# sjz5202/DisenLink

Measured on AMD Instinct MI355X. Metric: edges/sec (aggregate+score) at K=8 d=64, higher is better.
Workload: dtype f32; 1 GPU; squirrel_real (edge list of the parity fixture)(seed 0): N=5201, edge rows=217073, 85/5/10 split, E_sym=342129, scored train pairs P=1009603 (m=5), K=8, d=64, beta=0.5, t=1.0; forward route+aggregate+score_pairs; K=8, d=64, n_nodes=5201, E_sym=342129, P=1009603

## Files before the change

disenlink_amd/_lib.py:

```python
from __future__ import annotations

import ctypes as C
import os

PKG = os.path.dirname(os.path.abspath(__file__))
LIB_PATH = os.path.join(PKG, "libdisenlink_hip.so")


class DlCsrPlan(C.Structure):
    _fields_ = [
        ("n_rows", C.c_int32), ("row_offset", C.c_int32), ("n_total", C.c_int32), ("n_entries", C.c_int32),
        ("rowptr", C.c_void_p), ("col", C.c_void_p),
        ("seg_len", C.c_int32), ("n_seg", C.c_int32),
        ("seg_row", C.c_void_p), ("seg_beg", C.c_void_p), ("seg_end", C.c_void_p), ("seg_slot", C.c_void_p),
        ("n_slices", C.c_int32), ("slice_max_seg", C.c_int32), ("slice_seg0", C.c_void_p),
        ("n_multi", C.c_int32), ("n_slots", C.c_int32), ("multi_row", C.c_void_p), ("multi_slot0", C.c_void_p),
        ("slot_multi", C.c_void_p), ("unit_count", C.c_void_p),
    ]


class DlPairHub(C.Structure):
    _fields_ = [("n_blocks", C.c_int32), ("block_row", C.c_void_p),
                ("n_items", C.c_int32), ("n_slices", C.c_int32), ("slice_max_item", C.c_int32),
                ("slice_item0", C.c_void_p), ("item_block", C.c_void_p), ("item_step", C.c_void_p),
                ("n_steps", C.c_int32), ("step_v", C.c_void_p), ("step_u", C.c_void_p), ("step_q", C.c_void_p),
                ("step_q2", C.c_void_p), ("n_entries", C.c_int32),
                ("rest", DlCsrPlan), ("rest_pair", C.c_void_p), ("rest_pair2", C.c_void_p)]


class DlGraph(C.Structure):
    _fields_ = [("csr", DlCsrPlan), ("route", DlCsrPlan), ("rev", C.c_void_p), ("route_mirror", C.c_int32),
                ("route_hub", C.POINTER(DlPairHub))]


class DlPairIncidence(C.Structure):
    _fields_ = [("csr", DlCsrPlan), ("inc_pair", C.c_void_p), ("n_pairs", C.c_int32), ("entry_yw", C.c_void_p),
                ("inc_pair2", C.c_void_p), ("n_second", C.c_int32), ("hub", C.POINTER(DlPairHub))]


class DlHostCsr(C.Structure):
    _fields_ = [("n_nodes", C.c_int32), ("n_entries", C.c_int32), ("rowptr", C.POINTER(C.c_int32)),
                ("col", C.POINTER(C.c_int32)), ("rev", C.POINTER(C.c_int32))]


class DlHostPlan(C.Structure):
    _fields_ = [(n, C.c_int32) for n in ("seg_len", "n_seg", "n_slices", "slice_max_seg", "n_multi", "n_slots")] + \
               [(n, C.POINTER(C.c_int32)) for n in ("seg_row", "seg_beg", "seg_end", "seg_slot", "slice_seg0",
                                                    "multi_row", "multi_slot0", "slot_multi")]


class DlSparseFeatures(C.Structure):
    _fields_ = [("N", C.c_int32), ("F", C.c_int32), ("nnz", C.c_int32),
# ... 306 lines not shown
```

disenlink_amd/csrc/dl_api.hip:

```cpp
#include <stdarg.h>
#include <string.h>
#include "dl_common.h"
#include "dl_kernels.h"

namespace dl {

static thread_local char g_err[512] = "";
static int g_force_generic = 0;

void set_error(const char* fmt, ...) {
    va_list ap;
    va_start(ap, fmt);
    vsnprintf(g_err, sizeof(g_err), fmt, ap);
    va_end(ap);
}

int check_launch(const char* what) {
    hipError_t e = hipGetLastError();
    if (e != hipSuccess) {
        set_error("%s: %s", what, hipGetErrorString(e));
        return DL_E_LAUNCH;
    }
    return DL_OK;
}
// ... 258 lines not shown
static int score_pairs_fwd_space(const void* Z, const void* H, int N, int K, int d, dl_dtype dtype, float t,
                                 const int32_t* pu, const int32_t* pv, int n_pairs, const dl_pair_incidence* by_u,
                                 float* prob, float* coef, bool logit, void* stream) {
    if (int rc = check_shape(K, d)) return rc;
    if (int rc = check_dtype(by_u ? &by_u->csr : nullptr, K, d, dtype)) return rc;
    DL_REQUIRE(N >= 0 && n_pairs >= 0, "negative size");
    DL_REQUIRE(t != 0.0f, "temperature is 0");
    if (n_pairs == 0) return DL_OK;
    DL_REQUIRE(Z && H && pu && pv && prob, "NULL argument");
    if (by_u) {
        if (int rc = check_plan(&by_u->csr, "by_u")) return rc;
        const int n_second = by_u->inc_pair2 ? by_u->n_second : 0;
        DL_REQUIRE(n_second >= 0 && by_u->csr.n_entries + n_second == n_pairs && by_u->n_pairs == n_pairs && by_u->inc_pair,
                   "by_u must list each of the %d pairs exactly once", n_pairs);
        DL_REQUIRE(by_u->csr.n_total == N, "by_u.n_total=%d != N=%d", by_u->csr.n_total, N);
        if (const dl_pair_hub* hp = by_u->hub) {
            DL_REQUIRE(hp->n_items >= 0 && hp->n_entries >= 0 && hp->rest.n_entries >= 0 &&
                       hp->n_entries + hp->rest.n_entries == by_u->csr.n_entries,
                       "by_u.hub must hold each of the plan's %d entries exactly once", by_u->csr.n_entries);
            if (int rc = hp->n_items > 0 ? check_hub(hp, "by_u.hub", by_u->inc_pair2 != nullptr) : DL_OK) return rc;
            if (hp->rest.n_entries > 0) {
                if (int rc = check_plan(&hp->rest, "by_u.hub.rest")) return rc;
                DL_REQUIRE(hp->rest.n_total == N && hp->rest.seg_len == by_u->csr.seg_len && hp->rest_pair &&
                           (hp->rest_pair2 || !by_u->inc_pair2), "by_u.hub.rest does not match by_u");
            }
        }
        if (use_fast(&by_u->csr, K, d, dtype))
            return logit ? fast_score_pairs_logits_fwd(by_u, Z, H, K, d, dtype, t, prob, (hipStream_t)stream)
                         : fast_score_pairs_fwd(by_u, Z, H, K, d, dtype, t, prob, coef, (hipStream_t)stream);
    }
    DL_REQUIRE(coef == nullptr, "coef output needs the tuned scorer (a (K,d) with a fast path and a by_u plan)");
    if (logit)
        return generic_score_pairs_logits_fwd((const float*)Z, (const float*)H, K, d, t, pu, pv, n_pairs, prob,
                                              (hipStream_t)stream);
    return generic_score_pairs_fwd((const float*)Z, (const float*)H, K, d, t, pu, pv, n_pairs, prob,
                                   (hipStream_t)stream);
}

int dl_score_pairs_fwd(const void* Z, const void* H, int N, int K, int d, dl_dtype dtype, float t,
// ... 954 lines not shown
```

disenlink_amd/csrc/dl_config.h:

```cpp
#pragma once

namespace dl {

struct Config {
    int stream_rows;
    bool fwd_group_kernel;
    bool fwd_hub;
    bool route_hub;
    int auc_target;
    bool project_fp32_mfma;
    int fwd_groups;
    long long fwd_block_rows;
    long long bwd_block_bytes;
    int bwd_target;
    int inkernel_combine;
    int rank_slices;
    int mine_tiles;
    int sparse_seg;
};

const Config& config();
void config_reload();

}
// ... 1 lines not shown
```

disenlink_amd/csrc/dl_config.hip:

```cpp
#include <stdlib.h>
#include <algorithm>
#include <mutex>
#include "dl_config.h"
#include "disenlink_hip.h"

namespace dl {
namespace {

Config g_config;
std::once_flag g_once;

bool flag(const char* name) {
    const char* e = getenv(name);
    return e != nullptr && e[0] != '\0' && !(e[0] == '0' && e[1] == '\0');
}
long long number(const char* name) {
    const char* e = getenv(name);
    return e != nullptr && e[0] != '\0' ? atoll(e) : 0;
}

void read_environment() {
    Config c;
    const char* sr = getenv("DL_STREAM_ROWS");
    c.stream_rows = (sr == nullptr || sr[0] == '\0') ? -1 : (sr[0] == '1' ? 1 : 0);
    c.fwd_group_kernel = flag("DL_FWD_GROUP_KERNEL");
    const char* fh = getenv("DL_FWD_HUB");
    c.fwd_hub = !(fh != nullptr && fh[0] == '0' && fh[1] == '\0');
    const char* rh = getenv("DL_ROUTE_HUB");
    c.route_hub = !(rh != nullptr && rh[0] == '0' && rh[1] == '\0');
    c.auc_target = (int)std::max(0LL, number("DL_AUC_TARGET"));
    c.project_fp32_mfma = getenv("DL_PROJECT_FP32_MFMA") != nullptr;
    c.fwd_groups = (int)std::max(0LL, number("DL_FWD_GROUPS"));
    c.fwd_block_rows = std::max(0LL, number("DL_FWD_BLOCK_ROWS"));
    c.bwd_block_bytes = std::max(0LL, number("DL_BWD_BLOCK_BYTES"));
    c.bwd_target = (int)std::max(0LL, number("DL_BWD_TARGET"));
    const char* ic = getenv("DL_INKERNEL_COMBINE");
    c.inkernel_combine = (ic == nullptr || ic[0] == '\0') ? 1 : std::max(0, std::min(2, atoi(ic)));
    c.rank_slices = (int)std::max(0LL, number("DL_RANK_SLICES"));
    c.mine_tiles = (int)std::max(0LL, std::min(1LL << 20, number("DL_MINE_TILES")));
    c.sparse_seg = (int)std::max(0LL, std::min(1LL << 20, number("DL_SPARSE_SEG")));
    g_config = c;
}

}
// ... 15 lines not shown
```

disenlink_amd/csrc/dl_hub.h:

```cpp
#pragma once
#include "dl_fast.h"

namespace dl::fast::hub {
constexpr int WAVES = 8, THREADS = WAVES * DL_WAVE;
static_assert(DL_HUB_W == 2 * WAVES, "every wave stages two rows of the block");

typedef int dl_vi4 __attribute__((ext_vector_type(4)));
__device__ __forceinline__ dl_vi4 plan_words(const int32_t* a, int idx) {
    const auto* g = (const __attribute__((address_space(1))) int32_t*)a;
    return reinterpret_cast<const __attribute__((address_space(4))) dl_vi4*>((const __attribute__((address_space(4))) int32_t*)g)[idx];
}

template <bool ONE_STREAM>
__device__ __forceinline__ bool workgroup_item(const dl_pair_hub& h, int& it) {
    it = (int)blockIdx.x;
    if (ONE_STREAM && h.n_slices == 1) return it < h.n_items;
    const int x = blockIdx.x % h.n_slices;
    it = h.slice_item0[x] + (int)(blockIdx.x / h.n_slices);
    return it < h.slice_item0[x + 1];
}

struct ItemSteps { int a, b, c, end; };
__device__ __forceinline__ ItemSteps item_steps(const dl_pair_hub& h, int it) {
    return {h.item_step[4 * it], h.item_step[4 * it + 1], h.item_step[4 * it + 2], h.item_step[4 * it + 3]};
// ... 13 lines not shown
#pragma unroll
            for (int n = 0; n < NTAB; ++n) x[n] = dl_vf4{0.0f, 0.0f, 0.0f, 0.0f};
            if (row >= 0) {
#pragma unroll
                for (int n = 0; n < NTAB; ++n)
                    x[n] = *reinterpret_cast<const dl_vf4*>(tab[n] + (size_t)row * (NJ * 256) + (j * 64 + lane) * 4);
            }
#pragma unroll
            for (int n = 0; n < NTAB; ++n) urow[(ul * NTAB + n) * (NJ * 64) + j * 64 + lane] = x[n];
        }
    }
}

using FULL = std::false_type;
using LAST = std::true_type;
constexpr std::integral_constant<int, 4> SHAPE_A{};
constexpr std::integral_constant<int, 2> SHAPE_B{};
constexpr std::integral_constant<int, 1> SHAPE_C{};
template <typename Words, typename Fetch, typename Step>
__device__ __forceinline__ void walk(int s, const ItemSteps& st, Words nxt, Fetch&& fetch, Step&& step) {
    auto take = [&](const int cur) {
        const Words w = nxt;
        if (cur + WAVES < st.end) nxt = fetch(cur + WAVES);
        return w;
    };
    for (; s < st.b - 1; s += WAVES) step(take(s), s, SHAPE_A, FULL{});
    if (s == st.b - 1) step(take(s), s, SHAPE_A, LAST{}), s += WAVES;
    for (; s < st.c - 1; s += WAVES) step(take(s), s, SHAPE_B, FULL{});
    if (s == st.c - 1) step(take(s), s, SHAPE_B, LAST{}), s += WAVES;
    for (; s < st.end; s += WAVES) step(take(s), s, SHAPE_C, FULL{});
}

template <int NB, bool RARE_FLUSH>
struct Batch {
    int nb = 0;
    template <typename Flush, typename Open>
    __device__ __forceinline__ void tick(int step, Flush&& flush, Open&& open) {
        if (RARE_FLUSH ? __builtin_expect(nb == NB, 0) : nb == NB) {
            flush(), nb = 0, open(step + WAVES);
        }
    }
    template <typename Flush>
    __device__ __forceinline__ void close(Flush&& flush) { if (nb > 0) flush(); }
};
// ... 2 lines not shown
```

disenlink_amd/csrc/dl_score.h:

```cpp
#pragma once
#include "dl_fast.h"
#include "dl_hub.h"
#include "dl_score_bwd.h"

namespace dl {
namespace fast {

template <int K, int D, typename T, bool COEF, bool LOGIT = false>
__global__ __launch_bounds__(BLOCK, K <= 8 ? 4 : 1) void score_fwd_seg_kernel(dl_csr_plan g, const int32_t* __restrict__ pair_id,
                                                              const int32_t* __restrict__ pair_id2,
                                                              const T* __restrict__ Z, const T* __restrict__ H,
                                                              float t, float* __restrict__ prob,
                                                              float* __restrict__ coef_e,
                                                              float* __restrict__ coef_q) {
    using GE = Geo<K, D, T>;
    constexpr int VEC = GE::VEC, G = GE::G, EPW = GE::EPW, ROW = GE::ROW;
    constexpr int KB = K > 8 ? 8 : K;
    using FLB = FactorLanes<G, KB>;
    constexpr int KBP = FLB::KP;
    __shared__ __attribute__((aligned(16))) float urow[WAVES_PER_BLOCK][2 * ROW];
    const WaveSeg ws = load_wave_seg(g);
    const SegInfo si = ws.si;
    const int wave = ws.wave, lane = lane_id();
    const bool active = ws.active;
// ... 188 lines not shown
                 "v_add_f32_dpp %1, %5, %5 row_shl:4 row_mask:0xf bank_mask:0x5\n\t"
                 "v_add_f32_dpp %2, %6, %6 row_shl:4 row_mask:0xf bank_mask:0x5\n\t"
                 "v_add_f32_dpp %3, %7, %7 row_shl:4 row_mask:0xf bank_mask:0x5\n\t"
                 "v_add_f32_dpp %0, %8, %8 row_shr:4 row_mask:0xf bank_mask:0xa\n\t"
                 "v_add_f32_dpp %1, %9, %9 row_shr:4 row_mask:0xf bank_mask:0xa\n\t"
                 "v_add_f32_dpp %2, %10, %10 row_shr:4 row_mask:0xf bank_mask:0xa\n\t"
                 "v_add_f32_dpp %3, %11, %11 row_shr:4 row_mask:0xf bank_mask:0xa\n\t"
                 "s_nop 1"
                 : "=&v"(b[0]), "=&v"(b[1]), "=&v"(b[2]), "=&v"(b[3])
                 : "v"(a[0]), "v"(a[1]), "v"(a[2]), "v"(a[3]), "v"(a[4]), "v"(a[5]), "v"(a[6]), "v"(a[7]));
#pragma unroll
    for (int q = 0; q < 4; ++q) v[q] = b[q];
    TransposedReduce<4, 2>::run(v, c);
}

template <int K, int D, bool T1, bool COEF, bool FOLD, bool LOGIT = false>
__global__ __launch_bounds__(THREADS) __attribute__((amdgpu_waves_per_eu(4, 4))) void score_fwd_wave_kernel(
    dl_pair_hub h, const float* __restrict__ Z, const float* __restrict__ H, float t, float* __restrict__ prob,
    float* __restrict__ coef_e, float* __restrict__ coef_q) {
    using FW = FwdWave<K, D>;
    constexpr int NJ = FW::NJ, U = FW::U, ROW = K * D, R4 = 2 * ROW / 4;
    static_assert(D == 64 && NJ >= 1 && U == 4 && U * NJ <= 8, "the step geometry of score_fwd_wave_kernel");
    static_assert(!(LOGIT && COEF), "the logit form has no stored terms");
    constexpr bool BATCH = !COEF;
    __shared__ __attribute__((aligned(16))) float4 urow[DL_HUB_W * R4];
    int it;
    if (!workgroup_item<false>(h, it)) return;
    const int wave = wave_index(), lane = lane_id();
    const int i = lane & 15, r = lane >> 4;
    const int blk = h.item_block[it];
    const ItemSteps st = item_steps(h, it);
    stage_block<NJ, 2>((lds_vf4*)urow, h, blk, wave, lane, {Z, H});
    __syncthreads();
    auto fetch = [&](const int step) {
        const int s = __builtin_amdgcn_readfirstlane(step);
        StepWords w;
        w.v = plan_words(h.step_v, s), w.u = plan_words(h.step_u, s);
        w.q = w.p = dl_vi4{-1, -1, -1, -1};
        if constexpr (!BATCH) {
            w.q = plan_words(h.step_q, s);
            if constexpr (FOLD) w.p = plan_words(h.step_q2, s);
        }
        return w;
    };
    const int slot_step = lane >> 2;
    float lg = 0.0f;
// ... 1 lines not shown
    Batch<16, true> batch;
    auto open = [&](const int s0) {
        const int sb = s0 + WAVES * slot_step;
        pq = pq2 = -1;
        if (sb < st.end) {
            pq = h.step_q[4 * sb + (lane & 3)];
            if constexpr (FOLD) pq2 = h.step_q2[4 * sb + (lane & 3)];
        }
    };
    auto flush = [&]() {
        const float p = LOGIT ? lg : sigmoid_ref(lg);
        if (pq >= 0) prob[pq] = p;
        if (FOLD && pq2 >= 0) prob[pq2] = p;
    };
    auto do_step = [&](const StepWords& w, auto shape, auto last) {
        constexpr int NV = decltype(shape)::value;
        constexpr bool LAST = decltype(last)::value;
        const int sv[4] = {w.v.x, w.v.y, w.v.z, w.v.w}, su[4] = {w.u.x, w.u.y, w.u.z, w.u.w}, sq[4] = {w.q.x, w.q.y, w.q.z, w.q.w},
                  sq2[4] = {w.p.x, w.p.y, w.p.z, w.p.w};
        float4 zv[NV][NJ], hv[NV][NJ];
#pragma unroll
        for (int n = 0; n < NV; ++n) {
            if (!LAST || sv[n] >= 0) {
                const size_t v = (size_t)(unsigned)sv[n];
                const auto* zr = uniform_row<dl_vf4>(Z, v * ROW * sizeof(float));
                const auto* hr = uniform_row<dl_vf4>(H, v * ROW * sizeof(float));
#pragma unroll
                for (int j = 0; j < NJ; ++j) {
                    zv[n][j] = as_float4(zr[(unsigned)(lane + j * 64)]);
                    hv[n][j] = as_float4(hr[(unsigned)(lane + j * 64)]);
                }
// ... 4 lines not shown
        }
        float val[16];
#pragma unroll
        for (int q = 0; q < 16; ++q) val[q] = 0.0f;
#pragma unroll
        for (int j = 0; j < NJ; ++j) {
            float4 a4[U], b4[U];
#pragma unroll
            for (int e = 0; e < U; ++e) {
                const float4* mine = urow + (su[e] & (DL_HUB_W - 1)) * R4;
                a4[e] = mine[j * 64 + lane], b4[e] = mine[ROW / 4 + j * 64 + lane];
            }
            __builtin_amdgcn_sched_barrier(0);
#pragma unroll
            for (int e = 0; e < U; ++e) {
                val[j * 4 + e] = dot4_packed(a4[e], zv[e * NV / 4][j]);
                val[8 + j * 4 + e] = dot4_packed(b4[e], hv[e * NV / 4][j]);
            }
            __builtin_amdgcn_sched_barrier(0);
        }
        transposed_reduce16_masked(val, i);
        const float mine_v = val[0];
        const float ex = expf(T1 ? mine_v : mine_v / t);
        const float ttv = mine_v * xor_lane<8>(ex);
        float term = ttv;
        if constexpr (NJ == 2) term += xor_lane<4>(ttv);
        if constexpr (BATCH) {
            int tb = __float_as_int(term);
            tb = __builtin_amdgcn_update_dpp(tb, tb, 0x114, 0xF, 0x8, false);
            tb = __builtin_amdgcn_update_dpp(tb, tb, 0x128, 0xF, 0x3, false);
            const float logit = add_xor<32>(add_xor<16>(__int_as_float(tb)));
            lg = slot_step == batch.nb ? logit : lg;
// ... 183 lines not shown
                        if (coef) {
                            if (t == 1.0f) fold(std::true_type{}, std::true_type{}); else fold(std::false_type{}, std::true_type{});
                            return;
                        }
                    }
                    if (t == 1.0f) fold(std::true_type{}, std::false_type{}); else fold(std::false_type{}, std::false_type{});
                };
                auto wave_plan = [&](const dl_csr_plan* c, const int32_t* pair, const int32_t* pair2) {
                    pick([&](auto t1, auto cf, auto fo) {
                        hipLaunchKernelGGL((score_fwd_wave_kernel<K, D, decltype(t1)::value, decltype(cf)::value, decltype(fo)::value, LOGIT>),
                                           dim3(seg_blocks(c)), dim3(BLOCK), 0, st, *c, pair, pair2, (const float*)Z,
                                           (const float*)H, t, prob, coef, coef_q);
                    });
                };
                const dl_pair_hub* hp = config().fwd_hub ? by_u->hub : nullptr;
                if (hp != nullptr && hp->n_items > 0) {
                    pick([&](auto t1, auto cf, auto fo) {
                        hipLaunchKernelGGL((hub::score_fwd_wave_kernel<K, D, decltype(t1)::value, decltype(cf)::value, decltype(fo)::value, LOGIT>),
                                           dim3((unsigned)hp->n_slices * (unsigned)hp->slice_max_item), dim3(hub::THREADS), 0,
                                           st, *hp, (const float*)Z, (const float*)H, t, prob, coef, coef_q);
                    });
                    if (hp->rest.n_entries > 0) wave_plan(&hp->rest, hp->rest_pair, hp->rest_pair2);
                    return check_launch("score_pairs_fwd(fast, hub blocks + wave per entry)");
                }
                wave_plan(g, by_u->inc_pair, by_u->inc_pair2);
                return check_launch("score_pairs_fwd(fast, wave per entry)");
            }
        }
        if constexpr (!LOGIT) {
            if (coef) {
// ... 49 lines not shown
```

disenlink_amd/csrc/torch/dl_torch.cpp:

```cpp
#include <torch/library.h>
#include <torch/autograd.h>
#include <ATen/ATen.h>
#include <c10/hip/HIPStream.h>
#include "disenlink_hip.h"

#define DL_TORCH_BINDING_ABI 7

namespace {

using at::Tensor;
using torch::autograd::AutogradContext;
using torch::autograd::variable_list;

void check(int rc, const char* what) {
    TORCH_CHECK(rc == 0, what, " failed (", rc, "): ", dl_last_error());
}

void* stream() { return (void*)c10::hip::getCurrentHIPStream().stream(); }

template <bool LOGIT>
struct HotPathPairsLoss : public torch::autograd::Function<HotPathPairsLoss<LOGIT>> {
    static variable_list forward(AutogradContext* ctx, const Tensor& Z_in, int64_t graph_ptr, int64_t inc_ptr, int64_t n_edges,
                                 double beta, double t, const Tensor& label_in, const Tensor& weight_in, const Tensor& ws_g,
                                 const Tensor& ws_p, const Tensor& ws_b, int64_t table_bf16) {
// ... 277 lines not shown
```

disenlink_amd/graph.py:

```python
from __future__ import annotations

import os
import ctypes as C
import itertools
import weakref
from dataclasses import dataclass, field

import torch

from . import _lib

DEFAULT_SEG_LEN = int(os.environ.get("DL_SEG_LEN", "32"))
DEFAULT_ROUTE_SEG_LEN = int(os.environ.get("DL_ROUTE_SEG_LEN", "0"))


def route_seg_len(n_entries: int) -> int:
    if DEFAULT_ROUTE_SEG_LEN:
        return DEFAULT_ROUTE_SEG_LEN
    return 16 if n_entries >= 16 * 4096 else 8
DEFAULT_INC_SEG_LEN = 64
DEFAULT_RUN_LEN = 64
DEFAULT_SLICES = 8
UNIT_SEGS = 4
L2_BYTES_PER_XCD = 4 << 20
# ... 389 lines not shown
    pos = torch.arange(P, device=dev)
    occ = torch.empty(P, dtype=torch.int64, device=dev)
    occ[order] = pos - torch.cummax(torch.where(first, pos, torch.zeros_like(pos)), 0).values
    perm = torch.argsort((pu > pv).to(torch.int64), stable=True)
    perm = perm[torch.argsort(occ[perm], stable=True)]
    perm = perm[torch.argsort((lo_ * n_nodes + hi_)[perm], stable=True)]
    a, b = perm[:-1], perm[1:]
    match = (lo_[a] == lo_[b]) & (hi_[a] == hi_[b]) & (occ[a] == occ[b]) & (pu[a] < pv[a]) & (pu[b] > pv[b])
    second[a[match]] = b[match]
    return second


HUB_W = 16
HUB_MIN_SHARE = 1.25
HUB_ITEM_ROWS = 512


def hub_gathers(c: torch.Tensor) -> torch.Tensor:
    return c // 4 + torch.tensor([0, 1, 1, 2], device=c.device)[c % 4]


def hub_rank(row: torch.Tensor, n_nodes: int):
    cnt = torch.bincount(row, minlength=n_nodes)
    order = torch.argsort(-cnt, stable=True)
    rank = torch.empty_like(order)
    rank[order] = torch.arange(n_nodes, device=row.device)
    return rank, order, int((cnt > 0).sum())


def hub_block_counts(row: torch.Tensor, col: torch.Tensor, n_nodes: int):
    rank, _, n_live = hub_rank(row, n_nodes)
    nb = (n_live + HUB_W - 1) // HUB_W
    blk = torch.div(rank[row], HUB_W, rounding_mode="floor")
    key, c = torch.unique(blk * n_nodes + col, return_counts=True)
# ... 20 lines not shown
    n_slices: int
    slice_max_item: int
    slice_item0: torch.Tensor
    item_block: torch.Tensor
    item_slice: torch.Tensor
    item_step: torch.Tensor
    step_v: torch.Tensor
    step_u: torch.Tensor
    step_q: torch.Tensor
    step_q2: torch.Tensor | None
    n_entries: int
    rest: CsrPlan | None
    rest_pair: torch.Tensor | None
    rest_pair2: torch.Tensor | None
    _struct: _lib.DlPairHub | None = field(default=None, repr=False)

    @property
    def n_steps(self) -> int:
        return int(self.step_v.shape[0])

    @property
    def n_gathered(self) -> int:
        return int((self.step_v >= 0).sum())

    @staticmethod
    def build(row, col, pair, pair2, n_nodes: int, n_rows: int, n_slices: int, bounds, rest_csr,
              item_rows: int | None = None) -> "HubPlan":
        item_rows = HUB_ITEM_ROWS if item_rows is None else int(item_rows)
        dev = row.device
        ar = lambda n: torch.arange(n, device=dev)
        excl = lambda x: torch.cumsum(x, 0) - x
        rank, order, n_live = hub_rank(row, n_nodes)
        T = max(0, min(int(n_rows), n_live))
        nb = (T + HUB_W - 1) // HUB_W
# ... 75 lines not shown
        rest = rest_pair = rest_pair2 = None
        if int((~in_hub).sum()):
            got = rest_csr(~in_hub)
            rest, rest_pair = got[0], got[1]
            rest_pair2 = got[2] if len(got) > 2 else None
        item_block = torch.empty(I, dtype=torch.int64, device=dev)
        item_block[ipos] = i_blk
        item_slice = torch.empty(I, dtype=torch.int64, device=dev)
        item_slice[ipos] = i_sl
        item_step_s = torch.empty_like(item_step)
        item_step_s[ipos] = item_step
        return HubPlan(T, nb, _i32(block_row), I, n_streams, int(per_stream.max()) if I else 0, _i32(slice_item0),
                       _i32(item_block), _i32(item_slice), _i32(item_step_s), _i32(step_v), _i32(step_u), _i32(step_q),
                       None if step_q2 is None else _i32(step_q2), E, rest, rest_pair, rest_pair2)

    def to(self, device) -> "HubPlan":
        mv = lambda t: None if t is None else t.to(device)
        return HubPlan(self.n_rows, self.n_blocks, mv(self.block_row), self.n_items, self.n_slices, self.slice_max_item,
                       mv(self.slice_item0), mv(self.item_block), mv(self.item_slice), mv(self.item_step), mv(self.step_v),
                       mv(self.step_u), mv(self.step_q), mv(self.step_q2), self.n_entries, mv(self.rest),
                       mv(self.rest_pair), mv(self.rest_pair2))

    def check(self) -> None:
        if self.n_items == 0:
            return
        dev = self.step_v.device
        st = self.item_step.long()
        lens = torch.stack([st[:, 1] - st[:, 0], st[:, 2] - st[:, 1], st[:, 3] - st[:, 2]], dim=1).reshape(-1)
        ends = torch.cumsum(lens, 0)
        ok = bool((lens >= 0).all()) and int(ends[-1]) == self.n_steps and bool((st[1:, 0] == st[:-1, 3]).all()) \
            and int(st[0, 0]) == 0
        if ok:
            nv = torch.repeat_interleave(torch.tensor([4, 2, 1], device=dev).repeat(self.n_items), lens)
            last = torch.zeros(self.n_steps, dtype=torch.bool, device=dev)
            last[(ends - 1)[lens > 0]] = True
            used = torch.arange(4, device=dev)[None, :] < nv[:, None]
            live = (self.step_v >= 0) & used
            full = ~last | (nv == 1)
            ok = not bool(((used & ~live)[full]).any()) and bool(live[:, 0].all()) \
                and not bool((live[:, 1:] & ~live[:, :-1]).any())
        if not ok:
            raise ValueError("hub plan: dead partner rows may only close the last step of an item's A list and B list "
                             "(dl_pair_hub, disenlink_hip.h)")

    def c_value(self) -> _lib.DlPairHub:
        if self._struct is None:
            self.check()
            ptr = lambda t: None if t is None else t.data_ptr()
            self._struct = _lib.DlPairHub(
                self.n_blocks, ptr(self.block_row), self.n_items, self.n_slices, self.slice_max_item, ptr(self.slice_item0),
                ptr(self.item_block), ptr(self.item_step), self.n_steps, ptr(self.step_v), ptr(self.step_u),
                ptr(self.step_q), ptr(self.step_q2), self.n_entries,
                self.rest.c_value() if self.rest is not None else _lib.DlCsrPlan(), ptr(self.rest_pair), ptr(self.rest_pair2))
        return self._struct


ROUTE_HUB_ITEM_ROWS = 128
ROUTE_HUB_SLICES = 4


def route_hub_plan(row: torch.Tensor, col: torch.Tensor, rev: torch.Tensor, n_nodes: int, force: bool = False) -> HubPlan | None:
    e = torch.nonzero(col >= row).reshape(-1)
    if e.numel() == 0:
        return None
    r, c = row[e], col[e]
    deg = torch.bincount(row, minlength=n_nodes)
    swap = deg[c] > deg[r]
    owner, partner = torch.where(swap, c, r), torch.where(swap, r, c)
    e2 = rev[e]
# ... 7 lines not shown


@dataclass
class PairList(_PlanOwner):
    n_nodes: int
    pu: torch.Tensor
    pv: torch.Tensor
    by_u: CsrPlan
    by_u_pair: torch.Tensor
    inc: CsrPlan
    inc_pair: torch.Tensor
    fwd: CsrPlan | None = None
    fwd_pair: torch.Tensor | None = None
    fwd_pair2: torch.Tensor | None = None
    hub: HubPlan | None = None
    _struct: _lib.DlPairIncidence | None = field(default=None, repr=False)
    _struct_u: _lib.DlPairIncidence | None = field(default=None, repr=False)
    _yw: torch.Tensor | None = field(default=None, repr=False)
    _yw_key: tuple | None = field(default=None, repr=False)
    _yw_seen: tuple | None = field(default=None, repr=False)
    _ws_need: dict = field(default_factory=dict, repr=False)

    def __post_init__(self):
        _assign_handle(self)

    def bind_labels(self, label: torch.Tensor, weight: torch.Tensor, n_pairs_total: int | None = None) -> None:
        if os.environ.get("DL_ENTRY_LABELS", "1") == "0" or label.is_inference() or weight.is_inference():
            self.unbind_labels()
            return
        def same(key):
# ... 16 lines not shown

    def unbind_labels(self) -> None:
        self._yw = self._yw_key = None
        if self._struct is not None:
            self._struct.entry_yw = None

    @property
    def n_pairs(self) -> int:
        return int(self.pu.numel())

    @staticmethod
    def build(pu: torch.Tensor, pv: torch.Tensor, n_nodes: int, seg_len: int = DEFAULT_INC_SEG_LEN,
              run_len: int = DEFAULT_RUN_LEN, row_range: tuple[int, int] | None = None,
              n_slices: int | None = None, by_u_range: tuple[int, int] | None = None,
              build_by_u: bool = True, row_bytes: int = 2048, inc_slices: int | None = None,
              fold_mirrors: bool = True, hub_rows: int | None = None) -> "PairList":
        pu = pu.reshape(-1).to(torch.int64)
        pv = pv.reshape(-1).to(torch.int64)
        if pu.numel() != pv.numel():
            raise ValueError("pu and pv differ in length")
        P = pu.numel()
        if n_slices is None:
            n_slices = auto_slices(n_nodes, row_bytes, entries_per_row=P / max(1, len(torch.unique(pu))))
        if inc_slices is None:
            inc_slices = auto_inc_slices(n_nodes, row_bytes, entries_per_row=2.0 * P / max(1, n_nodes))
        if 2 * P >= 2 ** 31:
            raise ValueError("too many pairs for int32 incidence")
        if P and (int(torch.minimum(pu.min(), pv.min())) < 0 or int(torch.maximum(pu.max(), pv.max())) >= n_nodes):
            raise ValueError("pair endpoint outside [0, n_nodes)")
        dev = pu.device
        ids = torch.arange(P, device=dev)
# ... 29 lines not shown
            if bool((second >= 0).any()):
                kept = torch.ones(P, dtype=torch.bool, device=dev)
                kept[second[second >= 0]] = False
                f_u, f_v, f_q, f_q2 = pu[kept], pv[kept], ids[kept], second[kept]
                fwd, fwd_pair, fwd_pair2 = csr(f_u, f_v, f_q, ulo, uhi, run_len, unit_segs=1, pair2=f_q2)
        hub = None
        if hub_rows is not None and hub_rows > 0 and (by_u_range is not None or not build_by_u):
            raise ValueError("hub rows need the full-range forward plan")
        if build_by_u and by_u_range is None and P and hub_rows != 0:
            T = auto_hub_rows(f_u, f_v, n_nodes) if hub_rows is None else int(hub_rows)
            if T > 0:
                bnd = slice_bounds(f_v, n_slices) if n_slices > 1 else None
                rest_csr = lambda keep: csr(f_u[keep], f_v[keep], f_q[keep], 0, n_nodes, run_len, unit_segs=1,
                                            pair2=None if f_q2 is None else f_q2[keep], bnd=bnd)
                hub = HubPlan.build(f_u, f_v, f_q, f_q2, n_nodes, T, n_slices, bnd, rest_csr)
        return PairList(n_nodes, _i32(pu), _i32(pv), by_u, by_u_pair, inc, inc_pair, fwd, fwd_pair, fwd_pair2, hub)

    def c_struct(self, n_pairs_total: int | None = None):
        if self._struct is None:
            self._struct = _lib.DlPairIncidence(self.inc.c_value(), self.inc_pair.data_ptr(),
                                                self.n_pairs if n_pairs_total is None else n_pairs_total)
        return C.byref(self._struct)

    def c_struct_by_u(self):
        if self._struct_u is None:
            if self.fwd is None:
                self._struct_u = _lib.DlPairIncidence(self.by_u.c_value(), self.by_u_pair.data_ptr(), self.n_pairs)
            else:
                self._struct_u = _lib.DlPairIncidence(self.fwd.c_value(), self.fwd_pair.data_ptr(), self.n_pairs, None,
                                                      self.fwd_pair2.data_ptr(), self.n_pairs - self.fwd.n_entries)
            if self.hub is not None and self.hub.n_items > 0:
                self._struct_u.hub = C.pointer(self.hub.c_value())
        return C.byref(self._struct_u)

    def c_plan(self):
        self.c_struct()
        return C.byref(self._struct.csr)
```

disenlink_amd/native.py:

```python
from __future__ import annotations

import ctypes as C
import os

import torch

from . import _lib, ops
from .graph import Graph, PairList

LIB_PATH = os.path.join(os.path.dirname(os.path.abspath(__file__)), "libdisenlink_torch.so")
_state = {"loaded": None}
BINDING_ABI = 7
_OPS = ("hot_path_pairs_loss", "hot_path_pair_logits_loss", "project_stacked", "adam_step", "auc_pair_counts", "epoch_finish", "binding_abi")


def load() -> bool:
    if _state["loaded"] is None:
        ok = False
        if os.path.exists(LIB_PATH) and os.environ.get("DL_NATIVE_OPS", "1") != "0":
            _lib.load()
            try:
                torch.ops.load_library(LIB_PATH)
                ns = getattr(torch.ops, "disenlink_native", None)
                missing = [o for o in _OPS if ns is None or not hasattr(ns, o)]
                abi = None if missing else int(ns.binding_abi())
                ok = not missing and abi == BINDING_ABI
                if not ok:
# ... 70 lines not shown
```

include/disenlink_hip.h:

```cpp
#ifndef DISENLINK_HIP_H
#define DISENLINK_HIP_H

#include <stddef.h>
#include <stdint.h>

#ifdef __cplusplus
extern "C" {
#endif

#define DL_OK            0
#define DL_E_ARG        -1
#define DL_E_LAUNCH     -2
#define DL_E_WORKSPACE  -3

#define DL_MAX_FACTORS  64

typedef enum dl_dtype { DL_F32 = 0, DL_BF16 = 1 } dl_dtype;

#define DL_UNIT_SEGS 4
typedef struct dl_csr_plan {
    int32_t n_rows;
    int32_t row_offset;
    int32_t n_total;
    int32_t n_entries;
// ... 20 lines not shown
    dl_csr_plan csr;
    dl_csr_plan route;
    const int32_t* rev;
    int32_t route_mirror;
    const struct dl_pair_hub* route_hub;
} dl_graph;

typedef struct dl_pair_incidence {
    dl_csr_plan csr;
    const int32_t* inc_pair;
    int32_t n_pairs;
    const float* entry_yw;
    const int32_t* inc_pair2;
    int32_t n_second;
    const struct dl_pair_hub* hub;
} dl_pair_incidence;

#define DL_HUB_W 16
typedef struct dl_pair_hub {
    int32_t n_blocks;
    const int32_t* block_row;
    int32_t n_items;
    int32_t n_slices;
    int32_t slice_max_item;
    const int32_t* slice_item0;
    const int32_t* item_block;
    const int32_t* item_step;
    int32_t n_steps;
    const int32_t* step_v;
    const int32_t* step_u;
    const int32_t* step_q;
    const int32_t* step_q2;
    int32_t n_entries;
    dl_csr_plan rest;
    const int32_t* rest_pair;
    const int32_t* rest_pair2;
} dl_pair_hub;

typedef struct dl_host_csr {
    int32_t n_nodes;
    int32_t n_entries;
    int32_t* rowptr;
    int32_t* col;
    int32_t* rev;
} dl_host_csr;

typedef struct dl_host_plan {
    int32_t seg_len, n_seg, n_slices, slice_max_seg, n_multi, n_slots;
    int32_t *seg_row, *seg_beg, *seg_end, *seg_slot, *slice_seg0, *multi_row, *multi_slot0;
    int32_t* slot_multi;
} dl_host_plan;

// ... 357 lines not shown
```

Measured before the change: 9.145 billion edges/s.

## Add mixed-shape hub plan for pair scoring with degree-based pair ownership

Adds a second hub plan for the pair scorer. Each pair is owned by its higher-degree endpoint, so more pairs fall into the shared staged hub blocks. Leftover partner groups are packed into new 3+1 and 2+1+1 step shapes, which means fewer gather steps are wasted on dead slots. The scorer kernel gains a MIXED template that uses per-shape row maps, and it is launched by default when the mixed plan is present. The cost is more host-side planning, a changed ABI, and extra kernel variants.

```diff
diff --git a/disenlink_amd/_lib.py b/disenlink_amd/_lib.py
--- a/disenlink_amd/_lib.py
+++ b/disenlink_amd/_lib.py
@@ -28,6 +28,10 @@
                 ("rest", DlCsrPlan), ("rest_pair", C.c_void_p), ("rest_pair2", C.c_void_p)]
 
 
+class DlPairHubMixed(C.Structure):
+    _fields_ = [("hub", DlPairHub), ("n_lists", C.c_int32)]
+
+
 class DlGraph(C.Structure):
     _fields_ = [("csr", DlCsrPlan), ("route", DlCsrPlan), ("rev", C.c_void_p), ("route_mirror", C.c_int32),
                 ("route_hub", C.POINTER(DlPairHub))]
@@ -35,7 +39,8 @@
 
 class DlPairIncidence(C.Structure):
     _fields_ = [("csr", DlCsrPlan), ("inc_pair", C.c_void_p), ("n_pairs", C.c_int32), ("entry_yw", C.c_void_p),
-                ("inc_pair2", C.c_void_p), ("n_second", C.c_int32), ("hub", C.POINTER(DlPairHub))]
+                ("inc_pair2", C.c_void_p), ("n_second", C.c_int32), ("hub", C.POINTER(DlPairHub)),
+                ("hub_mixed", C.POINTER(DlPairHubMixed))]
 
 
 class DlHostCsr(C.Structure):
diff --git a/disenlink_amd/csrc/dl_api.hip b/disenlink_amd/csrc/dl_api.hip
--- a/disenlink_amd/csrc/dl_api.hip
+++ b/disenlink_amd/csrc/dl_api.hip
@@ -296,15 +296,22 @@
         DL_REQUIRE(n_second >= 0 && by_u->csr.n_entries + n_second == n_pairs && by_u->n_pairs == n_pairs && by_u->inc_pair,
                    "by_u must list each of the %d pairs exactly once", n_pairs);
         DL_REQUIRE(by_u->csr.n_total == N, "by_u.n_total=%d != N=%d", by_u->csr.n_total, N);
-        if (const dl_pair_hub* hp = by_u->hub) {
+        if (by_u->hub_mixed != nullptr)
+            DL_REQUIRE(by_u->hub_mixed->n_lists == DL_HUB_MIXED_LISTS, "by_u.hub_mixed: n_lists=%d, the kernels walk %d",
+                       by_u->hub_mixed->n_lists, DL_HUB_MIXED_LISTS);
+        const dl_pair_hub* const hubs[2] = {by_u->hub, by_u->hub_mixed ? &by_u->hub_mixed->hub : nullptr};
+        const char* const names[2][2] = {{"by_u.hub", "by_u.hub.rest"}, {"by_u.hub_mixed", "by_u.hub_mixed.rest"}};
+        for (int x = 0; x < 2; ++x) {
+            const dl_pair_hub* hp = hubs[x];
+            if (hp == nullptr) continue;
             DL_REQUIRE(hp->n_items >= 0 && hp->n_entries >= 0 && hp->rest.n_entries >= 0 &&
                        hp->n_entries + hp->rest.n_entries == by_u->csr.n_entries,
-                       "by_u.hub must hold each of the plan's %d entries exactly once", by_u->csr.n_entries);
-            if (int rc = hp->n_items > 0 ? check_hub(hp, "by_u.hub", by_u->inc_pair2 != nullptr) : DL_OK) return rc;
+                       "%s must hold each of the plan's %d entries exactly once", names[x][0], by_u->csr.n_entries);
+            if (int rc = hp->n_items > 0 ? check_hub(hp, names[x][0], by_u->inc_pair2 != nullptr) : DL_OK) return rc;
             if (hp->rest.n_entries > 0) {
-                if (int rc = check_plan(&hp->rest, "by_u.hub.rest")) return rc;
+                if (int rc = check_plan(&hp->rest, names[x][1])) return rc;
                 DL_REQUIRE(hp->rest.n_total == N && hp->rest.seg_len == by_u->csr.seg_len && hp->rest_pair &&
-                           (hp->rest_pair2 || !by_u->inc_pair2), "by_u.hub.rest does not match by_u");
+                           (hp->rest_pair2 || !by_u->inc_pair2), "%s does not match by_u", names[x][1]);
             }
         }
         if (use_fast(&by_u->csr, K, d, dtype))
diff --git a/disenlink_amd/csrc/dl_config.h b/disenlink_amd/csrc/dl_config.h
--- a/disenlink_amd/csrc/dl_config.h
+++ b/disenlink_amd/csrc/dl_config.h
@@ -7,6 +7,7 @@
     bool fwd_group_kernel;
     bool fwd_hub;
     bool route_hub;
+    bool score_hub_mixed;
     int auc_target;
     bool project_fp32_mfma;
     int fwd_groups;
diff --git a/disenlink_amd/csrc/dl_config.hip b/disenlink_amd/csrc/dl_config.hip
--- a/disenlink_amd/csrc/dl_config.hip
+++ b/disenlink_amd/csrc/dl_config.hip
@@ -28,6 +28,8 @@
     c.fwd_hub = !(fh != nullptr && fh[0] == '0' && fh[1] == '\0');
     const char* rh = getenv("DL_ROUTE_HUB");
     c.route_hub = !(rh != nullptr && rh[0] == '0' && rh[1] == '\0');
+    const char* hm = getenv("DL_SCORE_HUB_MIXED");
+    c.score_hub_mixed = !(hm != nullptr && hm[0] == '0' && hm[1] == '\0');
     c.auc_target = (int)std::max(0LL, number("DL_AUC_TARGET"));
     c.project_fp32_mfma = getenv("DL_PROJECT_FP32_MFMA") != nullptr;
     c.fwd_groups = (int)std::max(0LL, number("DL_FWD_GROUPS"));
diff --git a/disenlink_amd/csrc/dl_hub.h b/disenlink_amd/csrc/dl_hub.h
--- a/disenlink_amd/csrc/dl_hub.h
+++ b/disenlink_amd/csrc/dl_hub.h
@@ -51,9 +51,16 @@
 
 using FULL = std::false_type;
 using LAST = std::true_type;
-constexpr std::integral_constant<int, 4> SHAPE_A{};
-constexpr std::integral_constant<int, 2> SHAPE_B{};
-constexpr std::integral_constant<int, 1> SHAPE_C{};
+template <int NV, int R0, int R1, int R2, int R3>
+struct Shape {
+    static constexpr int value = NV;
+    static constexpr int row(int e) { return e == 0 ? R0 : e == 1 ? R1 : e == 2 ? R2 : R3; }
+};
+constexpr Shape<4, 0, 1, 2, 3> SHAPE_A{};
+constexpr Shape<2, 0, 0, 1, 1> SHAPE_B{};
+constexpr Shape<1, 0, 0, 0, 0> SHAPE_C{};
+constexpr Shape<3, 0, 0, 1, 2> SHAPE_A211{};
+constexpr Shape<2, 0, 0, 0, 1> SHAPE_B31{};
 template <typename Words, typename Fetch, typename Step>
 __device__ __forceinline__ void walk(int s, const ItemSteps& st, Words nxt, Fetch&& fetch, Step&& step) {
     auto take = [&](const int cur) {
@@ -65,6 +72,29 @@
     if (s == st.b - 1) step(take(s), s, SHAPE_A, LAST{}), s += WAVES;
     for (; s < st.c - 1; s += WAVES) step(take(s), s, SHAPE_B, FULL{});
     if (s == st.c - 1) step(take(s), s, SHAPE_B, LAST{}), s += WAVES;
+    for (; s < st.end; s += WAVES) step(take(s), s, SHAPE_C, FULL{});
+}
+
+struct MixedItemSteps { int a, a211, b, b31, c, end; };
+__device__ __forceinline__ MixedItemSteps mixed_item_steps(const dl_pair_hub& h, int it) {
+    return {h.item_step[6 * it],     h.item_step[6 * it + 1], h.item_step[6 * it + 2],
+            h.item_step[6 * it + 3], h.item_step[6 * it + 4], h.item_step[6 * it + 5]};
+}
+template <typename Words, typename Fetch, typename Step>
+__device__ __forceinline__ void walk(int s, const MixedItemSteps& st, Words nxt, Fetch&& fetch, Step&& step) {
+    auto take = [&](const int cur) {
+        const Words w = nxt;
+        if (cur + WAVES < st.end) nxt = fetch(cur + WAVES);
+        return w;
+    };
+    for (; s < st.a211 - 1; s += WAVES) step(take(s), s, SHAPE_A, FULL{});
+    if (s == st.a211 - 1) step(take(s), s, SHAPE_A, LAST{}), s += WAVES;
+    for (; s < st.b - 1; s += WAVES) step(take(s), s, SHAPE_A211, FULL{});
+    if (s == st.b - 1) step(take(s), s, SHAPE_A211, LAST{}), s += WAVES;
+    for (; s < st.b31 - 1; s += WAVES) step(take(s), s, SHAPE_B, FULL{});
+    if (s == st.b31 - 1) step(take(s), s, SHAPE_B, LAST{}), s += WAVES;
+    for (; s < st.c - 1; s += WAVES) step(take(s), s, SHAPE_B31, FULL{});
+    if (s == st.c - 1) step(take(s), s, SHAPE_B31, LAST{}), s += WAVES;
     for (; s < st.end; s += WAVES) step(take(s), s, SHAPE_C, FULL{});
 }
 
diff --git a/disenlink_amd/csrc/dl_score.h b/disenlink_amd/csrc/dl_score.h
--- a/disenlink_amd/csrc/dl_score.h
+++ b/disenlink_amd/csrc/dl_score.h
@@ -226,7 +226,7 @@
     TransposedReduce<4, 2>::run(v, c);
 }
 
-template <int K, int D, bool T1, bool COEF, bool FOLD, bool LOGIT = false>
+template <int K, int D, bool T1, bool COEF, bool FOLD, bool LOGIT = false, bool MIXED = false>
 __global__ __launch_bounds__(THREADS) __attribute__((amdgpu_waves_per_eu(4, 4))) void score_fwd_wave_kernel(
     dl_pair_hub h, const float* __restrict__ Z, const float* __restrict__ H, float t, float* __restrict__ prob,
     float* __restrict__ coef_e, float* __restrict__ coef_q) {
@@ -241,7 +241,10 @@
     const int wave = wave_index(), lane = lane_id();
     const int i = lane & 15, r = lane >> 4;
     const int blk = h.item_block[it];
-    const ItemSteps st = item_steps(h, it);
+    const std::conditional_t<MIXED, MixedItemSteps, ItemSteps> st = [&] {
+        if constexpr (MIXED) return mixed_item_steps(h, it);
+        else return item_steps(h, it);
+    }();
     stage_block<NJ, 2>((lds_vf4*)urow, h, blk, wave, lane, {Z, H});
     __syncthreads();
     auto fetch = [&](const int step) {
@@ -273,7 +276,8 @@
         if (FOLD && pq2 >= 0) prob[pq2] = p;
     };
     auto do_step = [&](const StepWords& w, auto shape, auto last) {
-        constexpr int NV = decltype(shape)::value;
+        using SH = decltype(shape);
+        constexpr int NV = SH::value;
         constexpr bool LAST = decltype(last)::value;
         const int sv[4] = {w.v.x, w.v.y, w.v.z, w.v.w}, su[4] = {w.u.x, w.u.y, w.u.z, w.u.w}, sq[4] = {w.q.x, w.q.y, w.q.z, w.q.w},
                   sq2[4] = {w.p.x, w.p.y, w.p.z, w.p.w};
@@ -308,8 +312,9 @@
             __builtin_amdgcn_sched_barrier(0);
 #pragma unroll
             for (int e = 0; e < U; ++e) {
-                val[j * 4 + e] = dot4_packed(a4[e], zv[e * NV / 4][j]);
-                val[8 + j * 4 + e] = dot4_packed(b4[e], hv[e * NV / 4][j]);
+                const int rw = MIXED ? SH::row(e) : e * NV / 4;
+                val[j * 4 + e] = dot4_packed(a4[e], zv[rw][j]);
+                val[8 + j * 4 + e] = dot4_packed(b4[e], hv[rw][j]);
             }
             __builtin_amdgcn_sched_barrier(0);
         }
@@ -523,6 +528,16 @@
                     });
                 };
                 const dl_pair_hub* hp = config().fwd_hub ? by_u->hub : nullptr;
+                const dl_pair_hub* hm = config().fwd_hub && config().score_hub_mixed && by_u->hub_mixed ? &by_u->hub_mixed->hub : nullptr;
+                if (hm != nullptr && hm->n_items > 0) {
+                    pick([&](auto t1, auto cf, auto fo) {
+                        hipLaunchKernelGGL((hub::score_fwd_wave_kernel<K, D, decltype(t1)::value, decltype(cf)::value, decltype(fo)::value, LOGIT, true>),
+                                           dim3((unsigned)hm->n_slices * (unsigned)hm->slice_max_item), dim3(hub::THREADS), 0,
+                                           st, *hm, (const float*)Z, (const float*)H, t, prob, coef, coef_q);
+                    });
+                    if (hm->rest.n_entries > 0) wave_plan(&hm->rest, hm->rest_pair, hm->rest_pair2);
+                    return check_launch("score_pairs_fwd(fast, mixed hub blocks + wave per entry)");
+                }
                 if (hp != nullptr && hp->n_items > 0) {
                     pick([&](auto t1, auto cf, auto fo) {
                         hipLaunchKernelGGL((hub::score_fwd_wave_kernel<K, D, decltype(t1)::value, decltype(cf)::value, decltype(fo)::value, LOGIT>),
diff --git a/disenlink_amd/csrc/torch/dl_torch.cpp b/disenlink_amd/csrc/torch/dl_torch.cpp
--- a/disenlink_amd/csrc/torch/dl_torch.cpp
+++ b/disenlink_amd/csrc/torch/dl_torch.cpp
@@ -4,7 +4,7 @@
 #include <c10/hip/HIPStream.h>
 #include "disenlink_hip.h"
 
-#define DL_TORCH_BINDING_ABI 7
+#define DL_TORCH_BINDING_ABI 8
 
 namespace {
 
diff --git a/disenlink_amd/graph.py b/disenlink_amd/graph.py
--- a/disenlink_amd/graph.py
+++ b/disenlink_amd/graph.py
@@ -427,10 +427,21 @@
 HUB_W = 16
 HUB_MIN_SHARE = 1.25
 HUB_ITEM_ROWS = 512
+HUB_SHAPES = ((0, 1, 2, 3), (0, 0, 1, 1), (0, 0, 0, 0))
+HUB_MIXED_SHAPES = ((0, 1, 2, 3), (0, 0, 1, 2), (0, 0, 1, 1), (0, 0, 0, 1), (0, 0, 0, 0))
+HUB_MIXED_OWNER = True
+HUB_MIXED_SHAPES_ON = True
+HUB_MIXED_ITEM_ROWS = 320
 
 
 def hub_gathers(c: torch.Tensor) -> torch.Tensor:
     return c // 4 + torch.tensor([0, 1, 1, 2], device=c.device)[c % 4]
+
+
+def hub_owner(row: torch.Tensor, col: torch.Tensor, n_nodes: int):
+    deg = torch.bincount(torch.cat([row, col]), minlength=n_nodes)
+    swap = (deg[col] > deg[row]) | ((deg[col] == deg[row]) & (col < row))
+    return torch.where(swap, col, row), torch.where(swap, row, col)
 
 
 def hub_rank(row: torch.Tensor, n_nodes: int):
@@ -481,10 +492,19 @@
     rest_pair: torch.Tensor | None
     rest_pair2: torch.Tensor | None
     _struct: _lib.DlPairHub | None = field(default=None, repr=False)
+    _struct_mixed: _lib.DlPairHubMixed | None = field(default=None, repr=False)
 
     @property
     def n_steps(self) -> int:
         return int(self.step_v.shape[0])
+
+    @property
+    def mixed(self) -> bool:
+        return int(self.item_step.shape[1]) == len(HUB_MIXED_SHAPES) + 1
+
+    @property
+    def shapes(self):
+        return HUB_MIXED_SHAPES if self.mixed else HUB_SHAPES
 
     @property
     def n_gathered(self) -> int:
@@ -590,6 +610,141 @@
                        _i32(item_block), _i32(item_slice), _i32(item_step_s), _i32(step_v), _i32(step_u), _i32(step_q),
                        None if step_q2 is None else _i32(step_q2), E, rest, rest_pair, rest_pair2)
 
+    @staticmethod
+    def build_mixed(row, col, pair, pair2, n_nodes: int, n_rows: int, n_slices: int, bounds, rest_csr,
+                    item_rows: int | None = None, mixed: bool = True) -> "HubPlan":
+        item_rows = HUB_ITEM_ROWS if item_rows is None else int(item_rows)
+        dev = row.device
+        ar = lambda n: torch.arange(n, device=dev)
+        excl = lambda x: torch.cumsum(x, 0) - x
+        rank, order, n_live = hub_rank(row, n_nodes)
+        T = max(0, min(int(n_rows), n_live))
+        nb = (T + HUB_W - 1) // HUB_W
+        block_row = torch.full((nb * HUB_W,), -1, dtype=torch.int64, device=dev)
+        block_row[:T] = order[:T]
+        in_hub = rank[row] < T
+        hrow, v, q = row[in_hub], col[in_hub], pair[in_hub]
+        q2 = None if pair2 is None else pair2[in_hub]
+        E = int(v.numel())
+        blk = torch.div(rank[hrow], HUB_W, rounding_mode="floor")
+        ul = rank[hrow] - blk * HUB_W
+        sl = torch.bucketize(v, bounds.to(dev), right=True) if n_slices > 1 else torch.zeros_like(v)
+        n_streams = min(n_slices, DEFAULT_SLICES)
+        key = (blk * n_slices + sl) * n_nodes + v
+        perm = torch.argsort(key, stable=True)
+        key, v, ul, q = key[perm], v[perm], ul[perm], q[perm]
+        q2 = None if q2 is None else q2[perm]
+        gnew = torch.ones(E, dtype=torch.bool, device=dev)
+        gnew[1:] = key[1:] != key[:-1]
+        gfirst = torch.nonzero(gnew).reshape(-1)
+        g_of = torch.cumsum(gnew, 0) - 1
+        G = int(gfirst.numel())
+        c = torch.bincount(g_of, minlength=G)
+        g_bs = torch.div(key[gfirst], n_nodes, rounding_mode="floor")
+        nC, rem = torch.div(c, 4, rounding_mode="floor"), c % 4
+        gath = nC + (rem > 0).long() if mixed else hub_gathers(c)
+        bs_new = torch.ones(G, dtype=torch.bool, device=dev)
+        bs_new[1:] = g_bs[1:] != g_bs[:-1]
+        bs_first = torch.nonzero(bs_new).reshape(-1)
+        bs_of = torch.cumsum(bs_new, 0) - 1
+        cum = excl(gath)
+        part = torch.div(cum - cum[bs_first][bs_of], item_rows, rounding_mode="floor")
+        inew = bs_new.clone()
+        inew[1:] |= part[1:] != part[:-1]
+        ifirst = torch.nonzero(inew).reshape(-1)
+        i_of = torch.cumsum(inew, 0) - 1
+        I = int(ifirst.numel())
+        tot = lambda at, x: torch.zeros(I, dtype=torch.int64, device=dev).index_add_(0, at, x)
+        cC, nC_i = excl(nC) - excl(nC)[ifirst][i_of], tot(i_of, nC)
+        if mixed:
+            pg = torch.nonzero(rem > 0).reshape(-1)
+            psz, poff = rem[pg], 4 * nC[pg]
+        else:
+            g2, g1 = torch.nonzero(rem >= 2).reshape(-1), torch.nonzero((rem == 1) | (rem == 3)).reshape(-1)
+            pg = torch.cat([g2, g1])
+            psz = torch.cat([torch.full_like(g2, 2), torch.ones_like(g1)])
+            poff = torch.cat([4 * nC[g2], 4 * nC[g1] + 2 * (rem[g1] == 3).long()])
+            o = torch.argsort(pg * 2 + (psz == 1).long(), stable=True)
+            pg, psz, poff = pg[o], psz[o], poff[o]
+        Pn = int(pg.numel())
+        pit = i_of[pg]
+
+        def ranked(size):
+            m = (psz == size).long()
+            n = tot(pit, m)
+            return n, excl(m) - excl(n)[pit]
+        (n1, k1), (n2, k2), (n3, k3) = ranked(1), ranked(2), ranked(3)
+        m31 = torch.minimum(n3, n1)
+        x3, r1 = n3 - m31, n1 - m31
+        nB, odd2 = torch.div(n2, 2, rounding_mode="floor"), n2 % 2
+        s211 = odd2 * torch.clamp(r1, max=2) if mixed else torch.zeros_like(r1)
+        lens = torch.stack([(r1 - s211 + 3) // 4, (s211 > 0).long(), nB + odd2 * (s211 == 0).long(), m31 + (x3 > 0).long(),
+                            nC_i + torch.clamp(x3 - 1, min=0)], dim=1)
+        n_i = lens.sum(1)
+        i_blk = torch.div(g_bs[ifirst], n_slices, rounding_mode="floor")
+        i_sl = g_bs[ifirst] - i_blk * n_slices
+        big = int(n_i.max()) + 1 if I else 1
+        iperm = torch.argsort(((i_sl % n_streams) * (n_slices + 1) + i_sl) * big + (big - 1 - n_i), stable=True)
+        ipos = torch.empty_like(iperm)
+        ipos[iperm] = ar(I)
+        base = torch.empty(I, dtype=torch.int64, device=dev)
+        base[iperm] = excl(n_i[iperm])
+        item_step = torch.cat([base[:, None], base[:, None] + torch.cumsum(lens, 1)], dim=1)
+        per_stream = torch.bincount(i_sl % n_streams, minlength=n_streams)
+        slice_item0 = torch.zeros(n_streams + 1, dtype=torch.int64, device=dev)
+        slice_item0[1:] = torch.cumsum(per_stream, 0)
+        S = int(n_i.sum())
+        LA, LA211, LB, LB31, LC = range(5)
+        m31p, s211p, nBp = m31[pit], s211[pit], nB[pit]
+        j1 = k1 - m31p
+        in31, in211, jA = k1 < m31p, (k1 >= m31p) & (j1 < s211p), j1 - s211p
+        last2 = k2 == 2 * nBp
+        w = torch.where
+        is1, is2 = psz == 1, psz == 2
+        p_list = w(is1, w(in31, LB31, w(in211, LA211, LA)), w(is2, w(last2 & (s211p > 0), LA211, LB), w(k3 <= m31p, LB31, LC)))
+        p_step = w(is1, w(in31, k1, w(in211, 0, torch.div(jA, 4, rounding_mode="floor"))),
+                   w(is2, w(last2, w(s211p > 0, 0, nBp), torch.div(k2, 2, rounding_mode="floor")),
+                     w(k3 <= m31p, k3, nC_i[pit] + k3 - m31p - 1)))
+        p_slot = w(is1, w(in31, 3, w(in211, 2 + j1, jA % 4)), w(is2 & ~last2, 2 * (k2 % 2), 0))
+        p_row = w(is1, w(in31, 1, w(in211, 1 + j1, jA % 4)), w(is2 & ~last2, k2 % 2, 0))
+        p_at = item_step[pit, p_list] + p_step
+        p = ar(E) - gfirst[g_of]
+        isC = p < 4 * nC[g_of]
+        g_piece = torch.full((G,), Pn, dtype=torch.int64, device=dev)
+        if Pn:
+            g_piece.scatter_reduce_(0, pg, ar(Pn), reduce="amin")
+        pe = torch.clamp(g_piece[g_of], max=max(Pn - 1, 0))
+        if not mixed and Pn:
+            pe = pe + (~isC & (p >= poff[pe] + psz[pe])).long()
+        if Pn == 0:
+            p_at = p_slot = p_row = poff = torch.zeros(1, dtype=torch.int64, device=dev)
+        step = w(isC, item_step[i_of[g_of], LC] + cC[g_of] + torch.div(p, 4, rounding_mode="floor"), p_at[pe])
+        slot = w(isC, p % 4, p_slot[pe] + p - poff[pe])
+        vset = w(isC, torch.zeros_like(p), p_row[pe])
+        mk = lambda fill: torch.full((S, 4), fill, dtype=torch.int64, device=dev)
+        step_v, step_u, step_q = mk(-1), mk(0), mk(-1)
+        step_v[step, vset] = v
+        step_u[step, slot] = ul
+        step_q[step, slot] = q
+        step_q2 = None
+        if q2 is not None:
+            step_q2 = mk(-1)
+            step_q2[step, slot] = q2
+        rest = rest_pair = rest_pair2 = None
+        if int((~in_hub).sum()):
+            got = rest_csr(~in_hub)
+            rest, rest_pair = got[0], got[1]
+            rest_pair2 = got[2] if len(got) > 2 else None
+        item_block = torch.empty(I, dtype=torch.int64, device=dev)
+        item_block[ipos] = i_blk
+        item_slice = torch.empty(I, dtype=torch.int64, device=dev)
+        item_slice[ipos] = i_sl
+        item_step_s = torch.empty_like(item_step)
+        item_step_s[ipos] = item_step
+        return HubPlan(T, nb, _i32(block_row), I, n_streams, int(per_stream.max()) if I else 0, _i32(slice_item0),
+                       _i32(item_block), _i32(item_slice), _i32(item_step_s), _i32(step_v), _i32(step_u), _i32(step_q),
+                       None if step_q2 is None else _i32(step_q2), E, rest, rest_pair, rest_pair2)
+
     def to(self, device) -> "HubPlan":
         mv = lambda t: None if t is None else t.to(device)
         return HubPlan(self.n_rows, self.n_blocks, mv(self.block_row), self.n_items, self.n_slices, self.slice_max_item,
@@ -602,22 +757,29 @@
             return
         dev = self.step_v.device
         st = self.item_step.long()
-        lens = torch.stack([st[:, 1] - st[:, 0], st[:, 2] - st[:, 1], st[:, 3] - st[:, 2]], dim=1).reshape(-1)
+        shapes = self.shapes
+        lens = (st[:, 1:] - st[:, :-1]).reshape(-1)
         ends = torch.cumsum(lens, 0)
-        ok = bool((lens >= 0).all()) and int(ends[-1]) == self.n_steps and bool((st[1:, 0] == st[:-1, 3]).all()) \
+        ok = bool((lens >= 0).all()) and int(ends[-1]) == self.n_steps and bool((st[1:, 0] == st[:-1, -1]).all()) \
             and int(st[0, 0]) == 0
         if ok:
-            nv = torch.repeat_interleave(torch.tensor([4, 2, 1], device=dev).repeat(self.n_items), lens)
+            smap = torch.repeat_interleave(torch.tensor(shapes, device=dev).repeat(self.n_items, 1), lens, dim=0)
+            nv = smap[:, 3] + 1
+            is_c = torch.repeat_interleave(torch.arange(len(shapes), device=dev).repeat(self.n_items), lens) == len(shapes) - 1
             last = torch.zeros(self.n_steps, dtype=torch.bool, device=dev)
             last[(ends - 1)[lens > 0]] = True
             used = torch.arange(4, device=dev)[None, :] < nv[:, None]
             live = (self.step_v >= 0) & used
-            full = ~last | (nv == 1)
+            full = ~last | is_c
             ok = not bool(((used & ~live)[full]).any()) and bool(live[:, 0].all()) \
                 and not bool((live[:, 1:] & ~live[:, :-1]).any())
+            if ok and self.mixed:
+                ok = not bool(((self.step_q >= 0) & ~torch.gather(live, 1, smap)).any())
         if not ok:
             raise ValueError("hub plan: dead partner rows may only close the last step of an item's A list and B list "
-                             "(dl_pair_hub, disenlink_hip.h)")
+                             "(dl_pair_hub, disenlink_hip.h)" if not self.mixed else
+                             "mixed hub plan: dead partner rows may only close the last step of an item's A, A211, B and B31 "
+                             "lists, and no live slot scores against one (dl_pair_hub_mixed, disenlink_hip.h)")
 
     def c_value(self) -> _lib.DlPairHub:
         if self._struct is None:
@@ -629,6 +791,13 @@
                 ptr(self.step_q), ptr(self.step_q2), self.n_entries,
                 self.rest.c_value() if self.rest is not None else _lib.DlCsrPlan(), ptr(self.rest_pair), ptr(self.rest_pair2))
         return self._struct
+
+    def c_value_mixed(self) -> _lib.DlPairHubMixed:
+        if self._struct_mixed is None:
+            if not self.mixed:
+                raise ValueError("not a mixed hub plan (HubPlan.build_mixed)")
+            self._struct_mixed = _lib.DlPairHubMixed(self.c_value(), len(HUB_MIXED_SHAPES))
+        return self._struct_mixed
 
 
 ROUTE_HUB_ITEM_ROWS = 128
@@ -666,6 +835,7 @@
     fwd_pair: torch.Tensor | None = None
     fwd_pair2: torch.Tensor | None = None
     hub: HubPlan | None = None
+    hub_mixed: HubPlan | None = None
     _struct: _lib.DlPairIncidence | None = field(default=None, repr=False)
     _struct_u: _lib.DlPairIncidence | None = field(default=None, repr=False)
     _yw: torch.Tensor | None = field(default=None, repr=False)
@@ -712,7 +882,7 @@
               run_len: int = DEFAULT_RUN_LEN, row_range: tuple[int, int] | None = None,
               n_slices: int | None = None, by_u_range: tuple[int, int] | None = None,
               build_by_u: bool = True, row_bytes: int = 2048, inc_slices: int | None = None,
-              fold_mirrors: bool = True, hub_rows: int | None = None) -> "PairList":
+              fold_mirrors: bool = True, hub_rows: int | None = None, hub_mixed: bool | None = None) -> "PairList":
         pu = pu.reshape(-1).to(torch.int64)
         pv = pv.reshape(-1).to(torch.int64)
         if pu.numel() != pv.numel():
@@ -772,7 +942,17 @@
                 rest_csr = lambda keep: csr(f_u[keep], f_v[keep], f_q[keep], 0, n_nodes, run_len, unit_segs=1,
                                             pair2=None if f_q2 is None else f_q2[keep], bnd=bnd)
                 hub = HubPlan.build(f_u, f_v, f_q, f_q2, n_nodes, T, n_slices, bnd, rest_csr)
-        return PairList(n_nodes, _i32(pu), _i32(pv), by_u, by_u_pair, inc, inc_pair, fwd, fwd_pair, fwd_pair2, hub)
+        mixed = None
+        if hub_mixed and hub is None:
+            raise ValueError("a mixed hub plan needs a list that gets a hub plan (hub_rows)")
+        if hub is not None and hub_mixed is not False:
+            o_u, o_v = hub_owner(f_u, f_v, n_nodes) if HUB_MIXED_OWNER else (f_u, f_v)
+            o_bnd = slice_bounds(o_v, n_slices) if n_slices > 1 else None
+            o_rest = lambda keep: csr(o_u[keep], o_v[keep], f_q[keep], 0, n_nodes, run_len, unit_segs=1,
+                                      pair2=None if f_q2 is None else f_q2[keep], bnd=o_bnd)
+            mixed = HubPlan.build_mixed(o_u, o_v, f_q, f_q2, n_nodes, n_nodes if hub_rows is None else T, n_slices, o_bnd,
+                                        o_rest, item_rows=HUB_MIXED_ITEM_ROWS, mixed=HUB_MIXED_SHAPES_ON)
+        return PairList(n_nodes, _i32(pu), _i32(pv), by_u, by_u_pair, inc, inc_pair, fwd, fwd_pair, fwd_pair2, hub, mixed)
 
     def c_struct(self, n_pairs_total: int | None = None):
         if self._struct is None:
@@ -788,7 +968,11 @@
                 self._struct_u = _lib.DlPairIncidence(self.fwd.c_value(), self.fwd_pair.data_ptr(), self.n_pairs, None,
                                                       self.fwd_pair2.data_ptr(), self.n_pairs - self.fwd.n_entries)
             if self.hub is not None and self.hub.n_items > 0:
+                if self.hub.mixed:
+                    raise ValueError("PairList.hub holds a mixed plan: that is PairList.hub_mixed")
                 self._struct_u.hub = C.pointer(self.hub.c_value())
+            if self.hub_mixed is not None and self.hub_mixed.n_items > 0:
+                self._struct_u.hub_mixed = C.pointer(self.hub_mixed.c_value_mixed())
         return C.byref(self._struct_u)
 
     def c_plan(self):
diff --git a/disenlink_amd/native.py b/disenlink_amd/native.py
--- a/disenlink_amd/native.py
+++ b/disenlink_amd/native.py
@@ -10,7 +10,7 @@
 
 LIB_PATH = os.path.join(os.path.dirname(os.path.abspath(__file__)), "libdisenlink_torch.so")
 _state = {"loaded": None}
-BINDING_ABI = 7
+BINDING_ABI = 8
 _OPS = ("hot_path_pairs_loss", "hot_path_pair_logits_loss", "project_stacked", "adam_step", "auc_pair_counts", "epoch_finish", "binding_abi")
 
 
diff --git a/include/disenlink_hip.h b/include/disenlink_hip.h
--- a/include/disenlink_hip.h
+++ b/include/disenlink_hip.h
@@ -58,6 +58,7 @@
     const int32_t* inc_pair2;
     int32_t n_second;
     const struct dl_pair_hub* hub;
+    const struct dl_pair_hub_mixed* hub_mixed;
 } dl_pair_incidence;
 
 #define DL_HUB_W 16
@@ -80,6 +81,12 @@
     const int32_t* rest_pair;
     const int32_t* rest_pair2;
 } dl_pair_hub;
+
+#define DL_HUB_MIXED_LISTS 5
+typedef struct dl_pair_hub_mixed {
+    dl_pair_hub hub;
+    int32_t n_lists;
+} dl_pair_hub_mixed;
 
 typedef struct dl_host_csr {
     int32_t n_nodes;
```

Result: faster. 10.18 billion edges/s (median of 6 runs) (+11.3%).
